# tomputer-g/SpatialVLA

Hardware: AMD Instinct MI355X
Metric: episodes/sec fwd+bwd SpatialVLA-4B, 224px+56tok batch, 1/2/4/8 MI355X (higher is better)
Workload: dtype bf16; 1 GPU; SpatialVLA-4B fwd+bwd+AdamW (BASELINE configs[2]/[3]); model=spatialvla_4b, global_batch=32, per_gpu_batch=32, seq_len=312, parallelism=dp1, trainable_params=3071421936

## Files before the change

### include/svla.h

```cpp
#ifndef SVLA_H_
#define SVLA_H_
#include <stddef.h>
#include <stdint.h>

#ifdef __cplusplus
extern "C" {
#endif

enum { SVLA_OK = 0, SVLA_ERR_ARG = 1, SVLA_ERR_HIP = 2 };

const char* svla_last_error(void);
const char* svla_version(void);

enum { SVLA_LAYOUT_KC = 0,
       SVLA_LAYOUT_RC = 1   };
enum { SVLA_SEG_OUTER = 0, SVLA_SEG_K = 1, SVLA_SEG_GEGLU = 2 };

typedef struct {
  const void* ptr[4];
  int64_t seg_start[5];
  int32_t nseg;
  int32_t seg_dim;
  int32_t layout;
  int32_t _pad;
// ... 199 lines not shown
                      int32_t patch, int32_t reso, int32_t n_freqs, void* feat, int64_t ldf, float* xyz_out,
                      void* stream);
int svla_inv3x3_f32(int32_t B, const float* K, float* kinv, void* stream);
int svla_im2col_patch(int32_t B, int32_t S, int32_t patch, const void* x, void* cols, int64_t ldc,
                      void* stream);
int svla_affine_bf16(int64_t n, const void* x, float scale, float offset, void* out, void* stream);
int svla_relu_fwd(int64_t n, const void* x, void* y, void* stream);
int svla_relu_bwd(int64_t n, const void* x, const void* dy, void* dx, void* stream);
int svla_geglu_bwd(int64_t M, int64_t I, const void* dh, int64_t ldh, const void* g, int64_t ldg, const void* u,
                   int64_t ldu, void* dg, int64_t lddg, void* du, int64_t lddu, void* stream);
int svla_geglu_bwd_mx(int64_t M, int64_t I, const void* dh, int64_t ldh, const void* g, int64_t ldg, const void* u,
                      int64_t ldu, void* dg, int64_t lddg, void* du, int64_t lddu, void* q, int64_t ldq, void* scales,
                      int64_t sld, void* stream);
int svla_add_bf16(int64_t n, const void* a, const void* b, void* out, void* stream);
int svla_gelu_rows(int64_t M, int64_t N, int32_t mode, const void* x, int64_t ldx, const void* pre, int64_t ldp,
                   void* y, int64_t ldy, void* stream);

int svla_gemv_rmsnorm2(int64_t M, int64_t N, int64_t K, const void* res, const void* y, int64_t ldx, const void* w1,
                       const void* w2, float eps1, float eps2, void* h_out, const svla_operand* B, void* c,
                       int64_t ldc, const svla_epilogue* epi, void* stream);
size_t svla_decode_mlp_sync_bytes(void);
int svla_decode_mlp_grid(int64_t M, int64_t H, int64_t I);
void svla_decode_mlp_debug(int grid_override, int cooperative, int timeout_ms);
int svla_decode_mlp(int64_t M, int64_t H, int64_t I, const void* res, void* y, int64_t ldx, const void* w1,
                    const void* w2, float eps1, float eps2, void* h_out, const void* w_gate, const void* w_up,
                    int64_t ldw, const void* w_down, int64_t ldd, void* act, int64_t ldact, void* out, int64_t ldo,
                    const void* attn, int64_t ld_attn, int64_t KO, const void* w_o, int64_t ldwo, unsigned* sync,
                    void* stream);

int svla_softcap_ce_rows(int64_t M, int64_t N, void* logits, int64_t ld, float cap, float* row_stats, void* stream);
int svla_ce_finalize(int64_t M, int64_t N, int64_t ntiles, const float* row_stats, const void* logits, int64_t ldl,
                     const int64_t* target, float* lse, int64_t* argmax, float* loss_rows, float* loss_out,
                     void* stream);
int svla_ce_bwd(int64_t M, int64_t N, const void* logits, int64_t ldl, const float* lse, const int64_t* target,
                float cap, const float* grad_scale, void* dlogits, int64_t ldd, void* stream);
int svla_action_accuracy(int64_t B, int64_t L, const int64_t* pred, int64_t ldp, const int64_t* labels, int64_t ldl,
                         const int64_t* ranges, int64_t* counts, float* acc, void* stream);

int svla_sumsq_bf16(int64_t n, const void* x, float* partial, int64_t n_partial, float* out, void* stream);
int svla_adamw(int64_t n, float* master, void* param_bf16, const void* grad_bf16, float* m, float* v, float lr,
               float beta1, float beta2, float eps, float weight_decay, float bc1, float bc2,
               const float* clip_scale, void* stream);
int svla_clip_scale(const float* sumsq, float max_norm, float* clip_scale, float* norm_out, void* stream);

int svla_zoe_attractor(int B, int H, int W, int n_att, int n_bins, const void* attractors, const int64_t* a_strides,
                       const void* centres, const int64_t* c_strides, float alpha, int gamma, int mean, void* out,
                       const int64_t* out_strides, void* stream);
int svla_zoe_readout_cat(int64_t B, int64_t T, int64_t C, const void* hidden, void* out, void* stream);
int svla_zoe_preprocess(int B, int C, int H, int W, int pad, int OH, int OW, const void* x, const float* mean,
                        const float* stdv, void* out, void* stream);
int svla_zoe_depth_resize(int B, int IH, int IW, int pad, int OH, int OW, const void* depth, void* out, void* stream);
int svla_upsample_bilinear_nhwc(int B, int C, int H1, int W1, int H2, int W2, int align_corners, float rh, float rw,
                                const void* in, void* out, void* stream);
int svla_zoe_metric_tail(int B, int H, int W, int h, int w, int CF, int CE, int NBins, int Hid,
                         const void* feat, const int64_t* feat_strides, const void* rel, const int64_t* rel_strides,
                         const void* emb, const int64_t* emb_strides, const void* ctr, const int64_t* ctr_strides,
                         const float* params, float p_eps, float max_t, float min_t, float clamp_eps, float* out,
                         void* stream);

enum { SVLA_CONV_PRE_RELU = 1, SVLA_CONV_POST_RELU = 2, SVLA_CONV_TRANSPOSED = 4 };
typedef struct {
  int32_t B, H, W, Cin;
  int32_t OH, OW, Cout;
  int32_t KH, KW, stride, pad;
  int32_t flags;
  int32_t factor;
// ... 17 lines not shown
```

### spatialvla_amd/_lib.py

```python
import ctypes
import os
import threading

import torch

_HERE = os.path.dirname(os.path.abspath(__file__))
LIB_PATH = os.environ.get("SVLA_LIB") or os.path.join(_HERE, "libsvla.so")

c_i64 = ctypes.c_int64
c_i32 = ctypes.c_int32
c_f32 = ctypes.c_float
c_vp = ctypes.c_void_p

LAYOUT_KC, LAYOUT_RC = 0, 1
SEG_OUTER, SEG_K, SEG_GEGLU = 0, 1, 2
(EPI_STORE, EPI_BIAS, EPI_BIAS_GELU, EPI_BIAS_RESID, EPI_GEGLU, EPI_GEGLU_BWD, EPI_GELU_BWD, EPI_SOFTCAP_CE, EPI_ROPE,
 EPI_BIAS_GELU_ERF, EPI_BIAS_SCALE_RESID) = range(11)


class Operand(ctypes.Structure):
    _fields_ = [("ptr", c_vp * 4), ("seg_start", c_i64 * 5), ("nseg", c_i32), ("seg_dim", c_i32),
                ("layout", c_i32), ("_pad", c_i32), ("ld", c_i64), ("r_valid", c_i64), ("k_valid", c_i64)]


# ... 99 lines not shown
    "svla_layernorm_bwd": (c_i32, [c_i64, c_i64, c_vp, c_vp, c_vp, c_vp, c_vp, c_vp, c_vp, c_vp,
                                   ctypes.POINTER(c_i64), c_vp]),
    "svla_colsum_f32": (c_i32, [c_i64, c_i64, c_vp, c_vp, c_i32, c_vp, c_vp]),
    "svla_rmsnorm2_bwd": (c_i32, [c_i64, c_i64] + [c_vp] * 11 + [ctypes.POINTER(c_i64), c_vp]),
    "svla_rmsnorm2_bwd_mx": (c_i32, [c_i64, c_i64] + [c_vp] * 11 + [ctypes.POINTER(c_i64), c_vp, c_i64, c_vp, c_i64,
                                                                    c_vp]),
    "svla_rmsnorm_bwd_mx": (c_i32, [c_i64, c_i64, c_vp, c_vp, c_vp, c_vp, c_vp, c_vp, c_vp, ctypes.POINTER(c_i64),
                                    c_vp, c_i64, c_vp, c_i64, c_vp]),
    "svla_colsum2_f32": (c_i32, [c_i64, c_i64, c_vp, c_vp, c_vp, c_i32, c_vp]),
    "svla_colsum_bf16": (c_i32, [c_i64, c_i64, c_vp, c_i64, c_vp, c_i32, c_vp, c_vp]),
    "svla_colsum_bf16_workspace_bytes": (ctypes.c_size_t, [c_i64, c_i64]),
    "svla_embed_merge": (c_i32, [c_i64, c_i64, c_vp, c_vp, c_vp, c_vp, c_i64, c_i64, c_vp, c_f32, c_vp, c_vp]),
    "svla_embed_merge_bwd": (c_i32, [c_i64, c_i64, c_vp, c_vp, c_vp, c_vp, c_i64, c_vp, c_f32, c_vp, c_vp, c_vp]),
    "svla_ego3d_encode": (c_i32, [c_i32, c_i32, c_i32, c_vp, c_vp, c_vp, c_i32, c_i32, c_i32, c_vp, c_i64, c_vp,
                                  c_vp]),
    "svla_inv3x3_f32": (c_i32, [c_i32, c_vp, c_vp, c_vp]),
    "svla_im2col_patch": (c_i32, [c_i32, c_i32, c_i32, c_vp, c_vp, c_i64, c_vp]),
    "svla_affine_bf16": (c_i32, [c_i64, c_vp, c_f32, c_f32, c_vp, c_vp]),
    "svla_relu_fwd": (c_i32, [c_i64, c_vp, c_vp, c_vp]),
    "svla_relu_bwd": (c_i32, [c_i64, c_vp, c_vp, c_vp, c_vp]),
    "svla_add_bf16": (c_i32, [c_i64, c_vp, c_vp, c_vp, c_vp]),
    "svla_gemv_rmsnorm2": (c_i32, [c_i64, c_i64, c_i64, c_vp, c_vp, c_i64, c_vp, c_vp, c_f32, c_f32, c_vp, c_vp,
                                   c_vp, c_i64, c_vp, c_vp]),
    "svla_decode_mlp_sync_bytes": (ctypes.c_size_t, []),
    "svla_decode_mlp_grid": (c_i32, [c_i64, c_i64, c_i64]),
    "svla_gemm_set_cu_cap": (None, [c_i32]),
    "svla_decode_mlp_debug": (None, [c_i32, c_i32, c_i32]),
    "svla_decode_mlp": (c_i32, [c_i64, c_i64, c_i64, c_vp, c_vp, c_i64, c_vp, c_vp, c_f32, c_f32, c_vp, c_vp, c_vp,
                                c_i64, c_vp, c_i64, c_vp, c_i64, c_vp, c_i64, c_vp, c_i64, c_i64, c_vp, c_i64, c_vp,
                                c_vp]),
    "svla_gelu_rows": (c_i32, [c_i64, c_i64, c_i32, c_vp, c_i64, c_vp, c_i64, c_vp, c_i64, c_vp]),
    "svla_softcap_ce_rows": (c_i32, [c_i64, c_i64, c_vp, c_i64, c_f32, c_vp, c_vp]),
    "svla_ce_finalize": (c_i32, [c_i64, c_i64, c_i64, c_vp, c_vp, c_i64, c_vp, c_vp, c_vp, c_vp, c_vp, c_vp]),
    "svla_ce_bwd": (c_i32, [c_i64, c_i64, c_vp, c_i64, c_vp, c_vp, c_f32, c_vp, c_vp, c_i64, c_vp]),
    "svla_conv2d_nhwc": (c_i32, [ctypes.POINTER(ConvArgs), c_vp]),
    "svla_action_accuracy": (c_i32, [c_i64, c_i64, c_vp, c_i64, c_vp, c_i64, ctypes.POINTER(c_i64), c_vp, c_vp,
                                     c_vp]),
    "svla_sumsq_bf16": (c_i32, [c_i64, c_vp, c_vp, c_i64, c_vp, c_vp]),
    "svla_adamw": (c_i32, [c_i64, c_vp, c_vp, c_vp, c_vp, c_vp, c_f32, c_f32, c_f32, c_f32, c_f32, c_f32, c_f32,
                           c_vp, c_vp]),
    "svla_clip_scale": (c_i32, [c_vp, c_f32, c_vp, c_vp, c_vp]),
    "svla_geglu_bwd": (c_i32, [c_i64, c_i64] + [c_vp, c_i64] * 5 + [c_vp]),
    "svla_geglu_bwd_mx": (c_i32, [c_i64, c_i64] + [c_vp, c_i64] * 7 + [c_vp]),
    "svla_upsample_bilinear_nhwc": (c_i32, [c_i32] * 7 + [c_f32, c_f32, c_vp, c_vp, c_vp]),
    "svla_zoe_readout_cat": (c_i32, [c_i64] * 3 + [c_vp] * 3),
    "svla_zoe_attractor": (c_i32, [c_i32] * 5 + [c_vp, ctypes.POINTER(c_i64), c_vp, ctypes.POINTER(c_i64), c_f32, c_i32,
                                   c_i32, c_vp, ctypes.POINTER(c_i64), c_vp]),
    "svla_zoe_preprocess": (c_i32, [c_i32] * 7 + [c_vp, ctypes.POINTER(c_f32), ctypes.POINTER(c_f32), c_vp, c_vp]),
    "svla_zoe_depth_resize": (c_i32, [c_i32] * 6 + [c_vp, c_vp, c_vp]),
    "svla_zoe_metric_tail": (c_i32, [c_i32] * 9 + [c_vp, ctypes.POINTER(c_i64)] * 4 + [c_vp] + [c_f32] * 4
                             + [c_vp, c_vp]),
}

_lock = threading.Lock()
_lib = None


class SvlaError(RuntimeError):
    pass


def load(path: str = LIB_PATH, strict: bool = True) -> ctypes.CDLL:
    if not os.path.exists(path):
        raise SvlaError(f"libsvla.so not found at {path}: build it with `python -c 'import __graft_entry__ as g; "
                        f"g.build()'` (make -C spatialvla_amd/csrc). There is no fallback path.")
    cdll = ctypes.CDLL(path, mode=ctypes.RTLD_GLOBAL)
# ... 23 lines not shown
```

### spatialvla_amd/csrc/gemm.hip

```cpp
#include "svla_common.h"
#include "agpr.h"
typedef int i32x8 __attribute__((ext_vector_type(8)));
#include "agpr_f8.h"
#include "softcap_tab.h"

#include <type_traits>

namespace {

constexpr int GELU_TAB_BYTES = sizeof(svla_gelu_bf16_tab);
static_assert(GELU_TAB_BYTES % 16 == 0, "table copied in 16-B pieces");
__device__ __forceinline__ void gelu_tab_to_lds(char* dst) {
  for (int t = threadIdx.x; t < GELU_TAB_BYTES / 16; t += blockDim.x)
    *(LDS_AS u32x4*)(dst + 16 * t) = reinterpret_cast<const u32x4*>(svla_gelu_bf16_tab)[t];
}

#ifndef G4_STAMPS
#define G4_STAMPS 0
#endif
#ifndef G4_GELU_LUT
#define G4_GELU_LUT 1
#endif
constexpr int BK = 64;
constexpr int GROUP_M = 8;
// ... 699 lines not shown
  op_setup<LA, BM, C::IA>(A, m0, rvA, w, lane, sa);
  op_setup<LB, BN, C::IB>(B, n0, rvB, w, lane, sb);

  constexpr int NLD = C::IA + C::IB;
  const int nk_all = (int)((K + BK - 1) / BK);
  const int kb = (C::NST > 2 && sp.S > 1) ? (int)((int64_t)split * nk_all / sp.S) : 0;
  const int nk = (C::NST > 2 && sp.S > 1) ? (int)((int64_t)(split + 1) * nk_all / sp.S) - kb : nk_all;
  auto mfma_stage = [&](const char* la) {
    const char* lb = la + C::A_BYTES;
#pragma unroll
    for (int ks = 0; ks < 2; ++ks) {
      bf16x8 af[TM], bfr[TN];
#pragma unroll
      for (int i = 0; i < TM; ++i) af[i] = read_frag<LA, BM>(la, C::WTM * wr + 16 * i, ks, lane);
#pragma unroll
      for (int j = 0; j < TN; ++j) bfr[j] = read_frag<LB, BN>(lb, C::WTN * wc + 16 * j, ks, lane);
#pragma unroll
      for (int i = 0; i < TM; ++i)
#pragma unroll
        for (int j = 0; j < TN; ++j) acc[i][j] = __builtin_amdgcn_mfma_f32_16x16x32_bf16(af[i], bfr[j], acc[i][j], 0, 0, 0);
    }
  };
  if constexpr (C::NST > 2) {
    constexpr int NST = C::NST;
#pragma unroll
    for (int st = 0; st < NST - 1; ++st)
      if (st < nk) {
        op_issue<LA, BM, C::IA>(A, sa, m0, (int64_t)(kb + st) * BK, kvA, smem + st * C::STAGE, w);
        op_issue<LB, BN, C::IB>(B, sb, n0, (int64_t)(kb + st) * BK, kvB, smem + st * C::STAGE + C::A_BYTES, w);
      }
#pragma unroll 1
    for (int kt = 0; kt < nk; ++kt) {
      vm_wait_upto<NLD, NST - 2>(min(NST - 2, nk - 1 - kt));
      __builtin_amdgcn_s_barrier();
      const int kn = kt + NST - 1;
      if (kn < nk) {
        char* dst = smem + (kn % NST) * C::STAGE;
        op_issue<LA, BM, C::IA>(A, sa, m0, (int64_t)(kb + kn) * BK, kvA, dst, w);
        op_issue<LB, BN, C::IB>(B, sb, n0, (int64_t)(kb + kn) * BK, kvB, dst + C::A_BYTES, w);
      }
      mfma_stage(smem + (kt % NST) * C::STAGE);
    }
    asm volatile("s_waitcnt lgkmcnt(0)" ::: "memory");
    __builtin_amdgcn_s_barrier();
    if (sp.S > 1) {
      const int tile = tm + tn * tiles_m;
      constexpr int SLAB = TM * TN * NTH * 16;
      const char* base = reinterpret_cast<const char*>(sp.slabs) + (int64_t)tile * sp.S * SLAB;
      {
        const __amdgpu_buffer_rsrc_t rs = make_rsrc(base + (int64_t)split * SLAB);
#pragma unroll
        for (int i = 0; i < TM; ++i)
#pragma unroll
          for (int j = 0; j < TN; ++j)
            __builtin_amdgcn_raw_buffer_store_b128(__builtin_bit_cast(u32x4, acc[i][j]), rs,
                                                   (uint32_t)((t + (i * TN + j) * NTH) * 16), 0, 16);
      }
      asm volatile("s_waitcnt vmcnt(0)" ::: "memory");
      __syncthreads();
      if (t == 0) {
        int* cnt = sp.counters + tile;
        const int old = __hip_atomic_fetch_add(cnt, 1, __ATOMIC_RELAXED, __HIP_MEMORY_SCOPE_AGENT);
        sflag = (old == sp.S - 1);
        if (old == sp.S - 1) __hip_atomic_store(cnt, 0, __ATOMIC_RELAXED, __HIP_MEMORY_SCOPE_AGENT);
      }
      __syncthreads();
// ... 2703 lines not shown
```

### spatialvla_amd/csrc/misc.hip

```cpp
#include "svla_common.h"

namespace {

bool al16(const void* p) { return ((uintptr_t)p & 15) == 0; }
inline unsigned nblk(int64_t n, int per) { return (unsigned)((n + per - 1) / per); }

__global__ void embed_merge_kernel(int64_t rows, int64_t H, const int64_t* __restrict__ ids,
                                   const int32_t* __restrict__ img_index, const bf16_t* __restrict__ embed,
                                   const bf16_t* __restrict__ spatial, int64_t a0, int64_t na,
                                   const bf16_t* __restrict__ img, float normalizer, bf16_t* __restrict__ out) {
  const int64_t row = blockIdx.x;
  const int64_t id = ids[row];
  const int ii = img_index ? img_index[row] : -1;
  const int64_t nch = H >> 3;
  for (int64_t ch = threadIdx.x; ch < nch; ch += blockDim.x) {
    float v[8];
    if (ii >= 0) {
      unpack8(*reinterpret_cast<const u32x4*>(img + (int64_t)ii * H + ch * 8), v);
    } else if (spatial && id >= a0 && id < a0 + na) {
      float e[8];
      unpack8(*reinterpret_cast<const u32x4*>(embed + id * H + ch * 8), e);
      unpack8(*reinterpret_cast<const u32x4*>(spatial + (id - a0) * H + ch * 8), v);
#pragma unroll
      for (int j = 0; j < 8; ++j) v[j] = round_bf(e[j] * 0.0f) + v[j];
// ... 569 lines not shown
                                 void* stream) {
  SVLA_CHECK_ARG(B > 0 && S % patch == 0 && x && cols && ldc >= 3 * patch * patch, "im2col: bad args");
  const int64_t rows = (int64_t)B * (S / patch) * (S / patch);
  hipLaunchKernelGGL(im2col_kernel, dim3((unsigned)rows), dim3(256), 0, (hipStream_t)stream, B, S, patch,
                     (const bf16_t*)x, (bf16_t*)cols, ldc);
  return svla::check_launch("im2col");
}

extern "C" int svla_affine_bf16(int64_t n, const void* x, float scale, float offset, void* out, void* stream) {
  SVLA_CHECK_ARG(n > 0 && x && out && al16(x) && al16(out), "affine: bad args");
  hipLaunchKernelGGL(affine_kernel, dim3(nblk(n, 256 * 8)), dim3(256), 0, (hipStream_t)stream, n, (const bf16_t*)x,
                     scale, offset, (bf16_t*)out);
  return svla::check_launch("affine");
}
extern "C" int svla_relu_fwd(int64_t n, const void* x, void* y, void* stream) {
  SVLA_CHECK_ARG(n > 0 && x && y, "relu: bad args");
  hipLaunchKernelGGL(relu_fwd_kernel, dim3(nblk(n, 256 * 8)), dim3(256), 0, (hipStream_t)stream, n,
                     (const bf16_t*)x, (bf16_t*)y);
  return svla::check_launch("relu_fwd");
}
extern "C" int svla_relu_bwd(int64_t n, const void* x, const void* dy, void* dx, void* stream) {
  SVLA_CHECK_ARG(n > 0 && x && dy && dx, "relu_bwd: bad args");
  hipLaunchKernelGGL(relu_bwd_kernel, dim3(nblk(n, 256 * 8)), dim3(256), 0, (hipStream_t)stream, n,
                     (const bf16_t*)x, (const bf16_t*)dy, (bf16_t*)dx);
  return svla::check_launch("relu_bwd");
}
extern "C" int svla_add_bf16(int64_t n, const void* a, const void* b, void* out, void* stream) {
  SVLA_CHECK_ARG(n > 0 && a && b && out && al16(a) && al16(b) && al16(out), "add: bad args");
  hipLaunchKernelGGL(add_kernel, dim3(nblk(n, 256 * 8)), dim3(256), 0, (hipStream_t)stream, n, (const bf16_t*)a,
                     (const bf16_t*)b, (bf16_t*)out);
  return svla::check_launch("add");
}

extern "C" int svla_ce_finalize(int64_t M, int64_t N, int64_t ntiles, const float* row_stats, const void* logits,
                                int64_t ldl, const int64_t* target, float* lse, int64_t* argmax, float* loss_rows,
                                float* loss_out, void* stream) {
  SVLA_CHECK_ARG(M > 0 && N > 0 && row_stats && logits && lse && argmax && loss_rows && loss_out, "ce_finalize: args");
  hipStream_t s = (hipStream_t)stream;
  hipLaunchKernelGGL(ce_finalize_kernel, dim3(nblk(M, 4)), dim3(256), 0, s, M, N, ntiles, row_stats,
                     (const bf16_t*)logits, ldl, target, lse, argmax, loss_rows);
  if (int rc = svla::check_launch("ce_finalize")) return rc;
  hipLaunchKernelGGL(ce_loss_kernel, dim3(1), dim3(1024), 0, s, M, loss_rows, target, loss_out);
  return svla::check_launch("ce_loss");
}

extern "C" int svla_ce_bwd(int64_t M, int64_t N, const void* logits, int64_t ldl, const float* lse,
                           const int64_t* target, float cap, const float* grad_scale, void* dlogits, int64_t ldd,
                           void* stream) {
  SVLA_CHECK_ARG(M > 0 && N > 0 && logits && lse && target && grad_scale && dlogits, "ce_bwd: args");
  SVLA_CHECK_ARG(ldl % 8 == 0 && ldd % 8 == 0 && ldd >= N, "ce_bwd: ld");
  dim3 grid(nblk(ldd, 256 * 8), (unsigned)M);
  hipLaunchKernelGGL(ce_bwd_kernel, grid, dim3(256), 0, (hipStream_t)stream, M, N, (const bf16_t*)logits, ldl, lse,
                     target, cap, grad_scale, (bf16_t*)dlogits, ldd);
  return svla::check_launch("ce_bwd");
}

extern "C" int svla_sumsq_bf16(int64_t n, const void* x, float* partial, int64_t n_partial, float* out,
                               void* stream) {
  SVLA_CHECK_ARG(n > 0 && x && partial && out && n_partial > 0 && n_partial <= 65535 && al16(x), "sumsq: args");
  hipStream_t s = (hipStream_t)stream;
  hipLaunchKernelGGL(sumsq_stage1, dim3((unsigned)n_partial), dim3(256), 0, s, n, (const bf16_t*)x, partial);
  if (int rc = svla::check_launch("sumsq1")) return rc;
  hipLaunchKernelGGL(sumsq_stage2, dim3(1), dim3(1024), 0, s, n_partial, partial, out);
  return svla::check_launch("sumsq2");
}

// ... 129 lines not shown
```

### spatialvla_amd/engine.py

```python
import math
from typing import Dict, List

import re

import torch
import torch.distributed as dist

from . import functional as Fn
from . import kernels as K

BF16 = torch.bfloat16


def _group_params(gmod) -> List[torch.nn.Parameter]:
    named = list(gmod.named_parameters())
    pmap = dict(named)
    out, done = [], set()
    for n, p in named:
        m = re.match(r"(.*self_attn\.)[qkv]_proj\.(weight|bias)$", n)
        if m is None:
            out.append(p)
            continue
        pre = m.group(1)
        if pre in done:
# ... 251 lines not shown
            dist.all_reduce(self.sumsq, op=dist.ReduceOp.SUM, group=ex.pg)
        Kx.clip_scale(self.sumsq, self.max_grad_norm, self.clip, self.gnorm)
        Fn.WEIGHT_EPOCH[0] += 1
        if self.overlap_opt:
            main = torch.cuda.current_stream(self.device)
            side = self._opt_stream
            side.wait_stream(main)
            with torch.cuda.stream(side):
                for b in self.opt_order:
                    ex.land(b)
                    o, c = ex.owned(b)
                    so = self.shard_offsets[b]
                    Kx.adamw(self.master[so:so + c], self.flat_param[o:o + c], self.flat_grad[o:o + c],
                             self.m[so:so + c], self.v[so:so + c], lr, self.betas[0], self.betas[1], self.eps,
                             self.wd, self.step_count, self.clip)
                    ex.all_gather(b)
                    ev = torch.cuda.Event()
                    ev.record(side)
                    self._opt_events[b] = ev
            return
        if self.world == 1:
            Kx.adamw(self.master, self.flat_param, self.flat_grad, self.m, self.v, lr, self.betas[0], self.betas[1],
                    self.eps, self.wd, self.step_count, self.clip)
            return
        for b in self.gather_order:
            ex.land(b)
            o, c = ex.owned(b)
            so = self.shard_offsets[b]
            Kx.adamw(self.master[so:so + c], self.flat_param[o:o + c], self.flat_grad[o:o + c], self.m[so:so + c],
                    self.v[so:so + c], lr, self.betas[0], self.betas[1], self.eps, self.wd, self.step_count, self.clip)
            ex.all_gather(b)

    def train_step(self, batch: Dict[str, torch.Tensor]):
        out = self.model(**batch, return_dict=True)
        self.synchronize()
        out.loss.backward()
        if batch.get("pixel_values") is None:
            for o, n in self.vision_slices:
                self.flat_grad[o:o + n].zero_()
        self.exchange.finish_reduce()
        self.optimizer_step()
        return out.loss.detach()

    def sync_params(self):
        self.synchronize()
        self.exchange.wait_all_params()

    def full_master(self) -> torch.Tensor:
        self.synchronize()
        ex = self.exchange
        if self.world == 1:
            return self.master.clone()
        out = torch.zeros(self.numel, dtype=torch.float32, device=self.device)
        for b, (s, e) in enumerate(self.buckets):
            so, c = self.shard_offsets[b], ex.chunk[b]
            parts = [torch.empty(c, dtype=torch.float32, device=self.device) for _ in range(self.world)]
            dist.all_gather(parts, self.master[so:so + c].contiguous(), group=ex.pg)
            out[s:e].copy_(torch.cat(parts))
        return out


def random_init_(model, seed: int = 0, std: float = 0.02):
    g = torch.Generator(device=next(model.parameters()).device)
    g.manual_seed(seed)
    with torch.no_grad():
        for n, p in model.named_parameters():
            if p.dim() >= 2:
# ... 8 lines not shown
```

### spatialvla_amd/functional.py

```python
import math
import os
import weakref
from dataclasses import dataclass
from typing import Optional

import torch

from . import _lib as L
from . import kernels as K

BF16 = torch.bfloat16
F32 = torch.float32


def _empty(*shape, dtype=BF16, like=None, device=None):
    return torch.empty(*shape, dtype=dtype, device=like.device if like is not None else device)


_FLAT_PARAMS: "weakref.WeakValueDictionary" = weakref.WeakValueDictionary()


def register_flat_param(p: torch.Tensor):
    _FLAT_PARAMS[(p.data_ptr(), tuple(p.shape))] = p

# ... 1156 lines not shown
        out = _empty(ids.numel(), H, like=embed_w)
        na = spatial_w.shape[0] if spatial_w is not None else 0
        K.embed_merge(ids, img_index, embed_w, spatial_w, a0, na, img_feats, normalizer, out)
        ctx.save_for_backward(ids, img_index, sort_rows, offsets, spatial_w, img_feats)
        ctx.normalizer, ctx.na = normalizer, na
        return out

    @staticmethod
    def backward(ctx, dout):
        ids, img_index, sort_rows, offsets, spatial_w, img_feats = ctx.saved_tensors
        dout = _c(dout)
        dimg = torch.empty_like(img_feats) if (img_feats is not None and ctx.needs_input_grad[2]) else None
        dsp, acc, rsp = (None, False, None)
        if spatial_w is not None and ctx.needs_input_grad[3]:
            dsp, acc, rsp = _grad_dest(spatial_w, True)
            if acc:
                tmp = torch.empty_like(spatial_w)
                K.embed_merge_bwd(ids, img_index, sort_rows, offsets, ctx.na, dout, ctx.normalizer, tmp, None)
                dsp.add_(tmp)
                dsp = None
        if dimg is not None or dsp is not None:
            K.embed_merge_bwd(ids, img_index, sort_rows, offsets, ctx.na, dout, ctx.normalizer, dsp, dimg)
        return None, None, dimg, rsp, None, None, None, None, None


class LMHeadCEFn(torch.autograd.Function):

    @staticmethod
    def forward(ctx, h, w, target, cap, stash):
        h = _c(h)
        M = h.shape[0]
        V = w.shape[0]
        ldv = K.round_up(V, 64)
        logits_buf = _empty(M, ldv, like=h)
        ntn = K.ceil_div(V, 128)
        stats = _empty(M, ntn, 3, dtype=F32, like=h)
        K.linear_fwd(h, [w], logits_buf[:, :V])
        K.softcap_ce_rows(logits_buf, V, stats, cap)
        lse = _empty(M, dtype=F32, like=h)
        argmax = _empty(M, dtype=torch.int64, like=h)
        loss_rows = _empty(M, dtype=F32, like=h)
        loss2 = _empty(2, dtype=F32, like=h)
        K.ce_finalize(V, ntn, stats, logits_buf[:, :V], target, lse, argmax, loss_rows, loss2)
        stash["argmax"] = argmax
        stash["lse"] = lse
        stash["n_valid"] = loss2[1:2]
        ctx.save_for_backward(h, w, logits_buf, lse, target, loss2)
        ctx.cap, ctx.V = cap, V
        ctx.row_plan = stash.pop("row_plan", None) if stash is not None else None
        ctx.mark_non_differentiable(logits_buf)
        ctx.set_materialize_grads(False)
        return logits_buf[:, :V], loss2[0]

    @staticmethod
    def backward(ctx, dlogits_unused, dloss):
        h, w, logits_buf, lse, target, loss2 = ctx.saved_tensors
        if dloss is None:
            return None, None, None, None, None
        M, ldv = logits_buf.shape
        V = ctx.V
        gscale = (dloss.float() / torch.clamp(loss2[1], min=1.0)).reshape(1).contiguous()
        if ctx.row_plan is not None:
            order, cnt, ev = ctx.row_plan
            if ev is not None:
                ev.synchronize()
                cnt = int(cnt[0])
            rows = order[:cnt]
        else:
            rows = torch.nonzero(target >= 0).view(-1)
        R = int(rows.numel())
        dh = torch.zeros_like(h) if ctx.needs_input_grad[0] else None
        dw, acc, rw = _grad_dest(w, ctx.needs_input_grad[1])
        if R == 0:
            if dw is not None and not acc:
                dw.zero_()
            return dh, rw, None, None, None
        dlog = _empty(R, ldv, like=h)
        K.ce_bwd(V, logits_buf.index_select(0, rows)[:, :V], lse.index_select(0, rows),
                 target.index_select(0, rows).contiguous(), ctx.cap, gscale, dlog)
        if dh is not None:
            dh_r = _empty(R, h.shape[1], like=h)
            A = K._operand([dlog], L.LAYOUT_KC, k_valid=ldv)
            Bop = K._operand([w], L.LAYOUT_RC, k_valid=V)
            K.gemm(R, w.shape[1], ldv, A, Bop, [dh_r], [0], dh_r.stride(0), K._epi(L.EPI_STORE))
            dh.index_copy_(0, rows, dh_r)
        if dw is not None:
            K.linear_wgrad(dlog[:, :V], h.index_select(0, rows).contiguous(), [dw], accumulate=acc)
        return dh, rw, None, None, None


def kv_class_from_additive_mask(mask: Optional[torch.Tensor], B: int, Lq: int, Lk: int, device) -> torch.Tensor:
# ... 113 lines not shown
```

### spatialvla_amd/kernels.py

```python
import ctypes
import os
import math
from typing import List, Optional, Sequence

import torch

from . import _lib as L

BF16 = torch.bfloat16


def _stream() -> int:
    return torch.cuda.current_stream().cuda_stream


def _ptr(t: Optional[torch.Tensor]):
    return None if t is None else t.data_ptr()


def _req(cond: bool, msg: str):
    if not cond:
        raise ValueError(msg)


# ... 785 lines not shown
    L.check(L.lib().svla_relu_bwd(x.numel(), x.data_ptr(), dy.data_ptr(), dx.data_ptr(), _stream()), "relu_bwd")


def add(a, b, out):
    L.check(L.lib().svla_add_bf16(a.numel(), a.data_ptr(), b.data_ptr(), out.data_ptr(), _stream()), "add")


GELU_TANH, GELU_ERF, GELU_TANH_BWD = 0, 1, 2


def gelu_rows(mode: int, x: torch.Tensor, y: torch.Tensor, pre: Optional[torch.Tensor] = None):
    _chk_bf16(x, "gelu_rows x")
    _chk_bf16(y, "gelu_rows y")
    M, N = x.shape
    _req(y.shape == x.shape and (pre is None or pre.shape == x.shape), "gelu_rows: shapes")
    L.check(L.lib().svla_gelu_rows(M, N, int(mode), x.data_ptr(), _ld(x), _ptr(pre), _ld(pre) if pre is not None else 0,
                                   y.data_ptr(), _ld(y), _stream()), "svla_gelu_rows")


def softcap_ce_rows(logits: torch.Tensor, N: int, row_stats: torch.Tensor, cap: float):
    _chk_bf16(logits, "softcap_ce_rows")
    M, ld = logits.shape[0], _ld(logits)
    _req(row_stats.dtype == torch.float32 and row_stats.is_contiguous() and row_stats.numel() >= M * ceil_div(N, 128) * 3,
         "softcap_ce_rows: row_stats must be a contiguous fp32 [M, ceil(N/128), 3]")
    L.check(L.lib().svla_softcap_ce_rows(M, N, logits.data_ptr(), ld, float(cap), row_stats.data_ptr(), _stream()),
            "svla_softcap_ce_rows")


def ce_finalize(N, ntiles, row_stats, logits, target, lse, argmax, loss_rows, loss_out):
    M = logits.shape[0]
    L.check(L.lib().svla_ce_finalize(M, N, ntiles, row_stats.data_ptr(), logits.data_ptr(), _ld(logits),
                                     _ptr(target), lse.data_ptr(), argmax.data_ptr(), loss_rows.data_ptr(),
                                     loss_out.data_ptr(), _stream()), "ce_finalize")


def ce_bwd(N, logits, lse, target, cap, grad_scale, dlogits):
    M = logits.shape[0]
    L.check(L.lib().svla_ce_bwd(M, N, logits.data_ptr(), _ld(logits), lse.data_ptr(), target.data_ptr(), cap,
                                grad_scale.data_ptr(), dlogits.data_ptr(), _ld(dlogits), _stream()), "ce_bwd")


def action_accuracy(pred: torch.Tensor, labels: torch.Tensor, ranges, counts=None, acc=None):
    B, Lp = pred.shape
    _req(labels.dim() == 2 and labels.shape[0] == B and Lp >= labels.shape[1] - 1, "action_accuracy: shapes")
    _req(pred.dtype == labels.dtype == torch.int64 and pred.is_cuda and labels.is_cuda, "action_accuracy: int64 CUDA")
    _req(pred.stride(1) == 1 and labels.stride(1) == 1, "action_accuracy: rows must be contiguous")
    if counts is None:
        counts = torch.empty(8, dtype=torch.int64, device=pred.device)
    if acc is None:
        acc = torch.empty(4, dtype=torch.float32, device=pred.device)
    rg = (ctypes.c_int64 * 6)(*[int(v) for v in ranges])
    L.check(L.lib().svla_action_accuracy(B, labels.shape[1], pred.data_ptr(), pred.stride(0), labels.data_ptr(),
                                         labels.stride(0), rg, counts.data_ptr(), acc.data_ptr(), _stream()),
            "svla_action_accuracy")
    return counts, acc


def sumsq(x_flat, out, n_partial=4096):
    part = torch.empty(n_partial, dtype=torch.float32, device=x_flat.device)
    L.check(L.lib().svla_sumsq_bf16(x_flat.numel(), x_flat.data_ptr(), part.data_ptr(), n_partial, out.data_ptr(),
                                    _stream()), "sumsq")


def clip_scale(sumsq_t, max_norm, clip, norm_out):
    L.check(L.lib().svla_clip_scale(sumsq_t.data_ptr(), max_norm, clip.data_ptr(), _ptr(norm_out), _stream()),
            "clip_scale")
# ... 297 lines not shown
```

### spatialvla_amd/modeling_spatialvla.py

```python
import os
import warnings
from dataclasses import dataclass
from typing import List, Optional, Tuple, Union

import torch
import torch.nn.functional as F
from torch import nn
from transformers import GenerationMixin, PreTrainedModel
from transformers.utils import ModelOutput

from . import functional as Fn
from . import zoe_fast

ZOE_STREAM = [os.environ.get("SVLA_ZOE_STREAM", "1") != "0"]
ZOE_STREAM_CAPTURE = [os.environ.get("SVLA_ZOE_STREAM_CAPTURE", "1") != "0"]
from . import kernels as K
from .configuration_spatialvla import SpatialVLAConfig
from .modeling_gemma2 import LORA_TARGETS, Gemma2ForCausalLM, Gemma2KVCache, KVMask, LoRAAdapter
from .modeling_siglip import SiglipVisionModel

SIGLIP_MEAN, SIGLIP_STD = (0.5, 0.5, 0.5), (0.5, 0.5, 0.5)
ZOE_MEAN, ZOE_STD = (0.5, 0.5, 0.5), (0.5, 0.5, 0.5)


# ... 87 lines not shown


class SpatialVLAForConditionalGeneration(SpatialVLAPreTrainedModel, GenerationMixin):
    def __init__(self, config: SpatialVLAConfig, vision_model=None, vision_zoe_model=None, projector_model=None,
                 language_model=None):
        super().__init__(config)
        self.vision_tower = vision_model or SiglipVisionModel(config.vision_config)
        self.multi_modal_projector = projector_model or SpatialVLAMultiModalProjector(config)
        self.vocab_size = config.text_config.vocab_size
        self.language_model = language_model or Gemma2ForCausalLM(config.text_config)
        if config.use_vision_zoe:
            from transformers import ZoeDepthForDepthEstimation
            self.vision_zoe_model = vision_zoe_model or ZoeDepthForDepthEstimation(config.vision_zoe_config)
            zoe_fast.install(self.vision_zoe_model)
            self.position_embedding_3d = Ego3DPositionEmbeddingMLP(
                config.ego3d_patch_reso ** 2 * 3, num_pos_feats=config.vision_config.hidden_size,
                n_freqs=config.n_freqs)
            patch_size, reso, image_size = (config.vision_config.patch_size, config.ego3d_patch_reso,
                                            config.vision_config.image_size)
            y, x = torch.meshgrid(torch.arange(0, image_size, patch_size // reso),
                                  torch.arange(0, image_size, patch_size // reso), indexing="ij")
            y, x = y + patch_size / reso / 2, x + patch_size / reso / 2
            uv_h = torch.stack([x, y, torch.ones_like(x)], dim=0).reshape(3, -1)
            self.register_buffer("uv_h", uv_h, persistent=False)
        if config.use_spatial_token:
            self.spatial_embed_tokens = nn.Embedding(config.spatial_token_num, config.text_config.hidden_size)
        else:
            self.spatial_embed_tokens = None
        self.pad_token_id = config.pad_token_id if config.pad_token_id is not None else -1
        self.decode_graphs = os.environ.get("SVLA_DECODE_GRAPHS", "1") != "0"
        self.strict_checks = True
        self.defer_checks = False
        self._deferred = []
        self.last_stash = {}
        self.post_init()

    @staticmethod
    def _pinned_i64(dev):
        return torch.zeros(1, dtype=torch.int64, pin_memory=dev.type == "cuda")

    def _defer(self, value, check):
        if value.device.type != "cuda" or not self.defer_checks:
            check(int(value))
            return
        buf = self._pinned_i64(value.device)
        buf.copy_(value.reshape(1).to(torch.int64), non_blocking=True)
        ev = torch.cuda.Event()
        ev.record()
        self._deferred.append((buf, ev, check))

    def check_deferred(self):
        pend, self._deferred = self._deferred, []
        for buf, ev, check in pend:
            ev.synchronize()
            check(int(buf[0]))

    def get_input_embeddings(self):
        return self.language_model.get_input_embeddings()

    def set_input_embeddings(self, value):
        self.language_model.set_input_embeddings(value)

    def get_output_embeddings(self):
        return self.language_model.get_output_embeddings()

    def set_output_embeddings(self, new_embeddings):
# ... 186 lines not shown
        attention_mask: Optional[torch.Tensor] = None,
        position_ids: Optional[torch.LongTensor] = None,
        past_key_values=None,
        token_type_ids: Optional[torch.LongTensor] = None,
        cache_position: Optional[torch.LongTensor] = None,
        inputs_embeds: Optional[torch.FloatTensor] = None,
        labels: Optional[torch.LongTensor] = None,
        use_cache: Optional[bool] = None,
        output_attentions: Optional[bool] = None,
        output_hidden_states: Optional[bool] = None,
        return_dict: Optional[bool] = None,
        num_logits_to_keep: int = 0,
        kv_mask: Optional[KVMask] = None,
    ) -> Union[Tuple, SpatialVLACausalLMOutputWithPast]:
        self.check_deferred()
        cache = past_key_values
        if cache is not None and not isinstance(cache, Gemma2KVCache):
            raise ValueError("past_key_values must be a Gemma2KVCache (see new_cache())")
        return_dict = True if return_dict is None else return_dict
        is_training = token_type_ids is not None and labels is not None
        if input_ids is None:
            if inputs_embeds is None:
                raise ValueError("forward needs input_ids (and optionally inputs_embeds)")
            if pixel_values is not None or self.config.use_spatial_token:
                raise ValueError("inputs_embeds without input_ids: the image and spatial-token merges need the ids")
        B, Lq = (input_ids if input_ids is not None else inputs_embeds).shape[:2]
        dev = (input_ids if input_ids is not None else inputs_embeds).device
        if cache is None and use_cache and not torch.is_grad_enabled():
            cache = self.new_cache(B, Lq + 256)
        if cache is not None:
            self._require_merged("forward(past_key_values=...)" if past_key_values is not None
                                 else "forward(use_cache=True) (it creates a KV cache)")

        image_features = None
        if pixel_values is not None:
            image_features = self.get_image_features(pixel_values, intrinsic)

        if labels is not None and input_ids is not None:
            has_pad = (labels == self.pad_token_id).any()
            labels = torch.where(has_pad & (input_ids == self.pad_token_id), -100, labels)

        if inputs_embeds is not None:
            hidden = self._merge_embeds(input_ids, inputs_embeds, image_features)
        else:
            hidden = self._merge_inputs(input_ids, image_features)
        past = cache.seen_tokens if cache is not None else 0
        if position_ids is None:
            start = past if cache_position is None else int(cache_position[0])
            position_ids = (torch.arange(start, start + Lq, device=dev) + 1)[None]
        if kv_mask is not None:
            mask = kv_mask
        elif past == 0:
            mask = KVMask.build(attention_mask, token_type_ids, is_training, B, Lq, dev)
        else:
            cls = torch.ones(B, Lq, dtype=torch.uint8, device=dev)
            if attention_mask is not None:
                cls = torch.where(attention_mask[:, -Lq:].to(dev) != 0, 1, 2).to(torch.uint8)
            mask = KVMask(cls.contiguous())
        attn_sink = [] if output_attentions else None
        h, all_h = self.language_model.model(hidden, mask, position_ids, output_hidden_states=bool(output_hidden_states),
                                             cache=cache, attn_sink=attn_sink)

        target = self._targets(labels, attention_mask, B, Lq, dev)
        stash = {}
        if labels is not None and torch.is_grad_enabled():
            stash["row_plan"] = self._label_rows(target)
        logits2d, loss = self.language_model.head(h, target, stash)
        self.last_stash = stash
        logits = logits2d.view(B, Lq, -1)
        if num_logits_to_keep:
            logits = logits[:, -num_logits_to_keep:]
        if labels is None:
            loss = None
        if not return_dict:
            out = (logits,)
            return (loss,) + out if loss is not None else out
        return SpatialVLACausalLMOutputWithPast(loss=loss, logits=logits, past_key_values=cache, hidden_states=all_h,
                                                attentions=tuple(attn_sink) if attn_sink is not None else None,
                                                image_hidden_states=image_features)

    def action_argmax(self):
        return self.last_stash.get("argmax")

    def action_token_ranges(self, action_tokenizer=None):
        at = action_tokenizer if action_tokenizer is not None else getattr(self, "action_tokenizer", None)
        if at is not None:
            return tuple(int(v) for t in (at.translation_tokenizer, at.rotation_tokenizer, at.gripper_tokenizer)
                         for v in (t.token_start_idx, t.token_end_idx))
        a0, n = int(self.config.action_token_begin_idx), int(self.config.spatial_token_num)
        if n != 8194:
            raise ValueError("action_token_ranges: pass the action tokenizer (non-canonical spatial_token_num)")
        return (a0, a0 + 4095, a0 + 4096, a0 + 8191, a0 + 8192, a0 + 8193)

    def action_metrics(self, labels: torch.Tensor, actions: Optional[torch.Tensor] = None, action_tokenizer=None,
                       argmax: Optional[torch.Tensor] = None):
        B, Lq = labels.shape
        am = argmax if argmax is not None else self.action_argmax()
        if am is None:
            raise ValueError("action_metrics: no argmax of a previous forward (run a training forward first)")
        am = am.view(B, -1)
        ranges = self.action_token_ranges(action_tokenizer)
        _counts, acc = K.action_accuracy(am, labels.contiguous(), ranges)
        out = {"accuracy": acc[0], "translation_accuracy": acc[1], "rotation_accuracy": acc[2],
# ... 464 lines not shown
```

Before: 150.0 episodes/s.

## Compute LM head and CE only on labeled rows during training

During train_step, the LM head projection, softcap cross-entropy and its backward run only on the rows that carry labels. Those rows are gathered with a new gather kernel, and the hidden-state gradient is scattered back into a zero-filled full-size buffer. This avoids computing full-vocabulary logits for all B*L positions when only the action tokens contribute to the loss. The cost is a host sync on the row count and no full logits returned in training. The diff also adds an lgkmcnt wait before the barrier in the GEMM main loop, which looks like a correctness fix.

```diff
diff --git a/include/svla.h b/include/svla.h
--- a/include/svla.h
+++ b/include/svla.h
@@ -255,6 +255,10 @@
 int svla_ce_finalize(int64_t M, int64_t N, int64_t ntiles, const float* row_stats, const void* logits, int64_t ldl,
                      const int64_t* target, float* lse, int64_t* argmax, float* loss_rows, float* loss_out,
                      void* stream);
+int svla_gather_rows_bf16(int64_t M, int64_t R, int64_t C, const int64_t* rows, const void* src, int64_t lds,
+                          void* dst, int64_t ldd, void* stream);
+int svla_scatter_rows_bf16(int64_t M, int64_t R, int64_t C, const int64_t* rows, const void* src, int64_t lds,
+                           void* dst, int64_t ldd, void* stream);
 int svla_ce_bwd(int64_t M, int64_t N, const void* logits, int64_t ldl, const float* lse, const int64_t* target,
                 float cap, const float* grad_scale, void* dlogits, int64_t ldd, void* stream);
 int svla_action_accuracy(int64_t B, int64_t L, const int64_t* pred, int64_t ldp, const int64_t* labels, int64_t ldl,
diff --git a/spatialvla_amd/_lib.py b/spatialvla_amd/_lib.py
--- a/spatialvla_amd/_lib.py
+++ b/spatialvla_amd/_lib.py
@@ -155,6 +155,8 @@
     "svla_gelu_rows": (c_i32, [c_i64, c_i64, c_i32, c_vp, c_i64, c_vp, c_i64, c_vp, c_i64, c_vp]),
     "svla_softcap_ce_rows": (c_i32, [c_i64, c_i64, c_vp, c_i64, c_f32, c_vp, c_vp]),
     "svla_ce_finalize": (c_i32, [c_i64, c_i64, c_i64, c_vp, c_vp, c_i64, c_vp, c_vp, c_vp, c_vp, c_vp, c_vp]),
+    "svla_gather_rows_bf16": (c_i32, [c_i64, c_i64, c_i64, c_vp, c_vp, c_i64, c_vp, c_i64, c_vp]),
+    "svla_scatter_rows_bf16": (c_i32, [c_i64, c_i64, c_i64, c_vp, c_vp, c_i64, c_vp, c_i64, c_vp]),
     "svla_ce_bwd": (c_i32, [c_i64, c_i64, c_vp, c_i64, c_vp, c_vp, c_f32, c_vp, c_vp, c_i64, c_vp]),
     "svla_conv2d_nhwc": (c_i32, [ctypes.POINTER(ConvArgs), c_vp]),
     "svla_action_accuracy": (c_i32, [c_i64, c_i64, c_vp, c_i64, c_vp, c_i64, ctypes.POINTER(c_i64), c_vp, c_vp,
diff --git a/spatialvla_amd/csrc/gemm.hip b/spatialvla_amd/csrc/gemm.hip
--- a/spatialvla_amd/csrc/gemm.hip
+++ b/spatialvla_amd/csrc/gemm.hip
@@ -755,6 +755,7 @@
 #pragma unroll 1
     for (int kt = 0; kt < nk; ++kt) {
       vm_wait_upto<NLD, NST - 2>(min(NST - 2, nk - 1 - kt));
+      asm volatile("s_waitcnt lgkmcnt(0)" ::: "memory");
       __builtin_amdgcn_s_barrier();
       const int kn = kt + NST - 1;
       if (kn < nk) {
diff --git a/spatialvla_amd/csrc/misc.hip b/spatialvla_amd/csrc/misc.hip
--- a/spatialvla_amd/csrc/misc.hip
+++ b/spatialvla_amd/csrc/misc.hip
@@ -625,6 +625,51 @@
   return svla::check_launch("add");
 }
 
+__global__ __launch_bounds__(256) void gather_rows_kernel(int64_t M, int64_t C8, const int64_t* __restrict__ rows,
+                                                          const u32x4* __restrict__ src, int64_t lds8,
+                                                          u32x4* __restrict__ dst, int64_t ldd8) {
+  const int64_t i = blockIdx.x, m = rows[i];
+  const bool ok = m >= 0 && m < M;
+  for (int64_t c = threadIdx.x; c < C8; c += blockDim.x)
+    dst[i * ldd8 + c] = ok ? src[m * lds8 + c] : u32x4{0u, 0u, 0u, 0u};
+}
+
+__global__ __launch_bounds__(256) void scatter_rows_kernel(int64_t R, int64_t C8, const int64_t* __restrict__ rows,
+                                                           const u32x4* __restrict__ src, int64_t lds8,
+                                                           u32x4* __restrict__ dst, int64_t ldd8) {
+  __shared__ int sidx;
+  const int64_t m = blockIdx.x;
+  if (threadIdx.x == 0) sidx = -1;
+  __syncthreads();
+  for (int64_t i = threadIdx.x; i < R; i += blockDim.x)
+    if (rows[i] == m) atomicMax(&sidx, (int)i);
+  __syncthreads();
+  const int i = sidx;
+  for (int64_t c = threadIdx.x; c < C8; c += blockDim.x)
+    dst[m * ldd8 + c] = i >= 0 ? src[(int64_t)i * lds8 + c] : u32x4{0u, 0u, 0u, 0u};
+}
+
+extern "C" int svla_gather_rows_bf16(int64_t M, int64_t R, int64_t C, const int64_t* rows, const void* src,
+                                     int64_t lds, void* dst, int64_t ldd, void* stream) {
+  SVLA_CHECK_ARG(M > 0 && R > 0 && R < ((int64_t)1 << 31) && C > 0 && rows && src && dst, "gather_rows: args");
+  SVLA_CHECK_ARG(C % 8 == 0 && lds % 8 == 0 && ldd % 8 == 0 && lds >= C && ldd >= C && al16(src) && al16(dst),
+                 "gather_rows: C, ld multiples of 8 elements, 16-B aligned pointers");
+  hipLaunchKernelGGL(gather_rows_kernel, dim3((unsigned)R), dim3(256), 0, (hipStream_t)stream, M, C / 8, rows,
+                     (const u32x4*)src, lds / 8, (u32x4*)dst, ldd / 8);
+  return svla::check_launch("gather_rows");
+}
+
+extern "C" int svla_scatter_rows_bf16(int64_t M, int64_t R, int64_t C, const int64_t* rows, const void* src,
+                                      int64_t lds, void* dst, int64_t ldd, void* stream) {
+  SVLA_CHECK_ARG(M > 0 && M < ((int64_t)1 << 31) && R > 0 && R < ((int64_t)1 << 31) && C > 0 && rows && src && dst,
+                 "scatter_rows: args");
+  SVLA_CHECK_ARG(C % 8 == 0 && lds % 8 == 0 && ldd % 8 == 0 && lds >= C && ldd >= C && al16(src) && al16(dst),
+                 "scatter_rows: C, ld multiples of 8 elements, 16-B aligned pointers");
+  hipLaunchKernelGGL(scatter_rows_kernel, dim3((unsigned)M), dim3(256), 0, (hipStream_t)stream, R, C / 8, rows,
+                     (const u32x4*)src, lds / 8, (u32x4*)dst, ldd / 8);
+  return svla::check_launch("scatter_rows");
+}
+
 extern "C" int svla_ce_finalize(int64_t M, int64_t N, int64_t ntiles, const float* row_stats, const void* logits,
                                 int64_t ldl, const int64_t* target, float* lse, int64_t* argmax, float* loss_rows,
                                 float* loss_out, void* stream) {
diff --git a/spatialvla_amd/engine.py b/spatialvla_amd/engine.py
--- a/spatialvla_amd/engine.py
+++ b/spatialvla_amd/engine.py
@@ -307,7 +307,11 @@
             ex.all_gather(b)
 
     def train_step(self, batch: Dict[str, torch.Tensor]):
-        out = self.model(**batch, return_dict=True)
+        prev, self.model.head_label_rows = getattr(self.model, "head_label_rows", False), True
+        try:
+            out = self.model(**batch, return_dict=True)
+        finally:
+            self.model.head_label_rows = prev
         self.synchronize()
         out.loss.backward()
         if batch.get("pixel_values") is None:
diff --git a/spatialvla_amd/functional.py b/spatialvla_amd/functional.py
--- a/spatialvla_amd/functional.py
+++ b/spatialvla_amd/functional.py
@@ -1212,6 +1212,10 @@
         M = h.shape[0]
         V = w.shape[0]
         ldv = K.round_up(V, 64)
+        rows = stash.pop("label_rows", None) if stash is not None else None
+        if rows is not None:
+            return LMHeadCEFn._forward_rows(ctx, h, w, target, cap, stash, rows)
+        ctx.rows_only = False
         logits_buf = _empty(M, ldv, like=h)
         ntn = K.ceil_div(V, 128)
         stats = _empty(M, ntn, 3, dtype=F32, like=h)
@@ -1233,10 +1237,61 @@
         return logits_buf[:, :V], loss2[0]
 
     @staticmethod
+    def _forward_rows(ctx, h, w, target, cap, stash, rows):
+        M, V = h.shape[0], w.shape[0]
+        R = int(rows.numel())
+        ldv = K.round_up(V, 64)
+        h_r = _empty(R, h.shape[1], like=h)
+        K.gather_rows(rows, h, h_r)
+        t_r = target.index_select(0, rows)
+        logits_r = _empty(R, ldv, like=h)
+        ntn = K.ceil_div(V, 128)
+        stats = _empty(R, ntn, 3, dtype=F32, like=h)
+        K.linear_fwd(h_r, [w], logits_r[:, :V])
+        K.softcap_ce_rows(logits_r, V, stats, cap)
+        lse_r = _empty(R, dtype=F32, like=h)
+        argmax_r = _empty(R, dtype=torch.int64, like=h)
+        loss_rows = _empty(R, dtype=F32, like=h)
+        loss2 = _empty(2, dtype=F32, like=h)
+        K.ce_finalize(V, ntn, stats, logits_r[:, :V], t_r, lse_r, argmax_r, loss_rows, loss2)
+        stash["argmax"] = torch.full((M,), -1, dtype=torch.int64, device=h.device).index_copy_(0, rows, argmax_r)
+        stash["lse"] = torch.full((M,), float("nan"), dtype=F32, device=h.device).index_copy_(0, rows, lse_r)
+        stash["n_valid"] = loss2[1:2]
+        stash.pop("row_plan", None)
+        ctx.save_for_backward(h_r, w, logits_r, lse_r, t_r, loss2, rows)
+        ctx.cap, ctx.V, ctx.M = cap, V, M
+        ctx.rows_only = True
+        ctx.set_materialize_grads(False)
+        return None, loss2[0]
+
+    @staticmethod
+    def _backward_rows(ctx, dloss):
+        h_r, w, logits_r, lse_r, t_r, loss2, rows = ctx.saved_tensors
+        R, ldv = logits_r.shape
+        V = ctx.V
+        gscale = (dloss.float() / torch.clamp(loss2[1], min=1.0)).reshape(1).contiguous()
+        dw, acc, rw = _grad_dest(w, ctx.needs_input_grad[1])
+        dlog = _empty(R, ldv, like=h_r)
+        K.ce_bwd(V, logits_r[:, :V], lse_r, t_r, ctx.cap, gscale, dlog)
+        dh = None
+        if ctx.needs_input_grad[0]:
+            dh_r = _empty(R, h_r.shape[1], like=h_r)
+            A = K._operand([dlog], L.LAYOUT_KC, k_valid=ldv)
+            Bop = K._operand([w], L.LAYOUT_RC, k_valid=V)
+            K.gemm(R, w.shape[1], ldv, A, Bop, [dh_r], [0], dh_r.stride(0), K._epi(L.EPI_STORE))
+            dh = _empty(ctx.M, h_r.shape[1], like=h_r)
+            K.scatter_rows(rows, dh_r, dh)
+        if dw is not None:
+            K.linear_wgrad(dlog[:, :V], h_r, [dw], accumulate=acc)
+        return dh, rw, None, None, None
+
+    @staticmethod
     def backward(ctx, dlogits_unused, dloss):
-        h, w, logits_buf, lse, target, loss2 = ctx.saved_tensors
         if dloss is None:
             return None, None, None, None, None
+        if ctx.rows_only:
+            return LMHeadCEFn._backward_rows(ctx, dloss)
+        h, w, logits_buf, lse, target, loss2 = ctx.saved_tensors
         M, ldv = logits_buf.shape
         V = ctx.V
         gscale = (dloss.float() / torch.clamp(loss2[1], min=1.0)).reshape(1).contiguous()
diff --git a/spatialvla_amd/kernels.py b/spatialvla_amd/kernels.py
--- a/spatialvla_amd/kernels.py
+++ b/spatialvla_amd/kernels.py
@@ -841,6 +841,29 @@
     L.check(L.lib().svla_ce_finalize(M, N, ntiles, row_stats.data_ptr(), logits.data_ptr(), _ld(logits),
                                      _ptr(target), lse.data_ptr(), argmax.data_ptr(), loss_rows.data_ptr(),
                                      loss_out.data_ptr(), _stream()), "ce_finalize")
+
+
+def _rows_args(rows, src, dst, what):
+    _chk_bf16(src, what)
+    _chk_bf16(dst, what)
+    _req(rows.dtype == torch.int64 and rows.dim() == 1 and rows.is_contiguous() and rows.numel() > 0,
+         f"{what}: rows must be a non-empty contiguous int64 vector")
+    _req(src.dim() == 2 and dst.dim() == 2 and src.shape[1] == dst.shape[1] and src.stride(1) == 1
+         and dst.stride(1) == 1, f"{what}: src / dst must be 2-D with the same contiguous columns")
+
+
+def gather_rows(rows: torch.Tensor, src: torch.Tensor, dst: torch.Tensor):
+    _rows_args(rows, src, dst, "gather_rows")
+    _req(dst.shape[0] == rows.numel(), "gather_rows: dst needs one row per entry of rows")
+    L.check(L.lib().svla_gather_rows_bf16(src.shape[0], rows.numel(), src.shape[1], rows.data_ptr(), src.data_ptr(),
+                                          _ld(src), dst.data_ptr(), _ld(dst), _stream()), "gather_rows")
+
+
+def scatter_rows(rows: torch.Tensor, src: torch.Tensor, dst: torch.Tensor):
+    _rows_args(rows, src, dst, "scatter_rows")
+    _req(src.shape[0] == rows.numel(), "scatter_rows: src needs one row per entry of rows")
+    L.check(L.lib().svla_scatter_rows_bf16(dst.shape[0], rows.numel(), src.shape[1], rows.data_ptr(), src.data_ptr(),
+                                           _ld(src), dst.data_ptr(), _ld(dst), _stream()), "scatter_rows")
 
 
 def ce_bwd(N, logits, lse, target, cap, grad_scale, dlogits):
diff --git a/spatialvla_amd/modeling_spatialvla.py b/spatialvla_amd/modeling_spatialvla.py
--- a/spatialvla_amd/modeling_spatialvla.py
+++ b/spatialvla_amd/modeling_spatialvla.py
@@ -143,6 +143,7 @@
         self.strict_checks = True
         self.defer_checks = False
         self._deferred = []
+        self.head_label_rows = False
         self.last_stash = {}
         self.post_init()
 
@@ -395,13 +396,17 @@
             self._require_merged("forward(past_key_values=...)" if past_key_values is not None
                                  else "forward(use_cache=True) (it creates a KV cache)")
 
+        if labels is not None and input_ids is not None:
+            has_pad = (labels == self.pad_token_id).any()
+            labels = torch.where(has_pad & (input_ids == self.pad_token_id), -100, labels)
+        target = self._targets(labels, attention_mask, B, Lq, dev)
+        stash = {}
+        if labels is not None and torch.is_grad_enabled():
+            stash["row_plan"] = self._label_rows(target)
+
         image_features = None
         if pixel_values is not None:
             image_features = self.get_image_features(pixel_values, intrinsic)
-
-        if labels is not None and input_ids is not None:
-            has_pad = (labels == self.pad_token_id).any()
-            labels = torch.where(has_pad & (input_ids == self.pad_token_id), -100, labels)
 
         if inputs_embeds is not None:
             hidden = self._merge_embeds(input_ids, inputs_embeds, image_features)
@@ -424,14 +429,17 @@
         h, all_h = self.language_model.model(hidden, mask, position_ids, output_hidden_states=bool(output_hidden_states),
                                              cache=cache, attn_sink=attn_sink)
 
-        target = self._targets(labels, attention_mask, B, Lq, dev)
-        stash = {}
-        if labels is not None and torch.is_grad_enabled():
-            stash["row_plan"] = self._label_rows(target)
+        if self.head_label_rows and "row_plan" in stash:
+            order, cnt, ev = stash["row_plan"]
+            if ev is not None:
+                ev.synchronize()
+                cnt = int(cnt[0])
+            if cnt > 0:
+                stash["label_rows"] = order[:cnt]
         logits2d, loss = self.language_model.head(h, target, stash)
         self.last_stash = stash
-        logits = logits2d.view(B, Lq, -1)
-        if num_logits_to_keep:
+        logits = logits2d.view(B, Lq, -1) if logits2d is not None else None
+        if num_logits_to_keep and logits is not None:
             logits = logits[:, -num_logits_to_keep:]
         if labels is None:
             loss = None
```

Result: faster. 158.3 episodes/s, median of 6 (+5.5%).
